# annihilatorrrr/spacedrive

Measured on AMD Instinct MI355X. Metric: cas_ids/sec + hashed GB/s (whole node), 10M files at 1/2/4/8 MI355X, higher is better.
Workload: dtype u32; 1 GPU; sampled-path cas_id (57,352-B BLAKE3 message/file) + Object grouping; 1310720 files/GPU/step (1310720 per step at n_gpus=1); dup_permille=300, parallelism=shard-by-file x1, grouping=fused

## Files before the change

spacedrive_amd/csrc/cas_hash.hip:

```cpp
#include <hip/hip_runtime.h>
#include <stdint.h>

#include "blake3_lane.hpp"
#include "blake3_tree.hpp"
#include "sd_dup_probe.h"
#include "sd_dup_runs.h"
#include "sd_group.h"
#include "sd_kernels.h"
#include "sd_mix.h"
#include "sd_ws.h"

namespace sdcas {


constexpr uint32_t SAMPLED_PAIRS = SAMPLED_CONTENT_LEN / 128;
constexpr uint32_t SAMPLED_CHUNKS = SAMPLED_CONTENT_LEN / 1024;
static_assert(SAMPLED_PAIRS == 8 * SAMPLED_CHUNKS, "the sampled content is whole chunks of 8 lines");

__device__ __forceinline__ void load_pair_here(const uint4* __restrict__ q, uint32_t P,
                                               uint4 (&buf)[8]) {
  __builtin_amdgcn_sched_barrier(0);
  line(q, P, buf);
  __builtin_amdgcn_sched_barrier(0);
}

constexpr int SAMPLED_DEPTH = 5;
constexpr int SAMPLED_BLOCK = 512;

template <int B = SAMPLED_BLOCK>
using LdsStack = CvStack<B, false>;

template <int BLK = SAMPLED_BLOCK>
__device__ __forceinline__ uint64_t cas_lane_sampled(const uint4* __restrict__ q, uint64_t size,
                                                     LdsStack<BLK>& stk) {
  uint4 A[8], B[8];
  uint32_t cv[8];
  auto push_chunk = [&](uint32_t total) { merge_push(stk, cv, total); };
// ... 136 lines not shown
  uint64_t key = 0;
  if (live) {
    LdsStack<B> stk{stack_lds, threadIdx.x};
    const uint4* q = reinterpret_cast<const uint4*>(content + f * stride);
    key = cas_lane_sampled<B>(q, sizes[f], stk);
  }
  if (blockIdx.x == 0 && threadIdx.x < 2) ro.objects[threadIdx.x] = 0;
  region_epilogue<B>(stack_lds, live, f, key, keys, ro);
}

extern "C" __global__ void __launch_bounds__(SAMPLED_BLOCK)
sd_cas_sampled_group_kernel(const uint8_t* __restrict__ content, uint64_t stride,
                            const uint64_t* __restrict__ sizes, uint64_t n,
                            uint64_t* __restrict__ keys, RegionOut ro) {
  sampled_group_kernel_body<SAMPLED_BLOCK>(content, stride, sizes, n, keys, ro);
}

extern "C" __global__ void __launch_bounds__(SAMPLED_BLOCK_NARROW)
sd_cas_sampled_group_kernel_256(const uint8_t* __restrict__ content, uint64_t stride,
                                const uint64_t* __restrict__ sizes, uint64_t n,
                                uint64_t* __restrict__ keys, RegionOut ro) {
  sampled_group_kernel_body<SAMPLED_BLOCK_NARROW>(content, stride, sizes, n, keys, ro);
}

struct DupLists {
  const uint32_t* cand;
  uint32_t* list_h;
  uint32_t* list_c;
  uint32_t* same;
  uint32_t* cnt;
  uint32_t* first;
  uint32_t* rank;
  uint32_t* counters;
  uint32_t tail_tiles;
  volatile uint32_t* note;
  uint32_t seq, files;
};
constexpr uint32_t DUP_N_HASH = 0, DUP_N_CAND = 1, DUP_VERIFIED = 2, DUP_REHASHED = 3, DUP_QUEUE = 4,
                   DUP_GROUPS = 5, DUP_TASKS = 6, DUP_REFS = 7;
static_assert(DUP_REFS < DUP_COUNTERS, "counters");

extern "C" __global__ void __launch_bounds__(256)
sd_dup_probe_kernel(const uint8_t* __restrict__ content, uint64_t stride,
                    const uint64_t* __restrict__ sizes, uint64_t n, uint64_t* __restrict__ probes,
                    uint32_t* __restrict__ counters, uint32_t* __restrict__ cnt) {
  const uint64_t f = (uint64_t)blockIdx.x * 256 + threadIdx.x;
  if (blockIdx.x == 0 && threadIdx.x < DUP_COUNTERS) counters[threadIdx.x] = 0;
  if (f < n) {
    probes[f] = dup_probe(sizes[f], content + f * stride);
    cnt[f] = 0;
  }
}

extern "C" __global__ void __launch_bounds__(256)
sd_dup_compact_kernel(uint64_t n, DupLists dl) {
  __shared__ uint32_t wcnt[3][4], base;
  const uint64_t f = (uint64_t)blockIdx.x * 256 + threadIdx.x;
  const uint32_t lane = threadIdx.x & 63u, w = threadIdx.x >> 6;
  const bool live = f < n;
  const uint32_t g = live ? dl.cand[f] : 0u;
  const bool h = live && g == (uint32_t)f;
  const bool c = live && !h;
  uint32_t r = 1;
  if (c) {
    r = atomicAdd(&dl.cnt[g], 1u);
    dl.rank[f] = r;
  }
  const uint64_t bh = __ballot(h), bc = __ballot(c), bg = __ballot(r == 0);
  const uint64_t below = (1ull << lane) - 1ull;
  if (lane == 0) {
    wcnt[0][w] = (uint32_t)__popcll(bh);
    wcnt[1][w] = (uint32_t)__popcll(bc);
    wcnt[2][w] = (uint32_t)__popcll(bg);
  }
  __syncthreads();
  if (threadIdx.x < 3) {
    constexpr uint32_t word[3] = {DUP_N_HASH, DUP_N_CAND, DUP_GROUPS};
    const uint32_t t = wcnt[threadIdx.x][0] + wcnt[threadIdx.x][1] + wcnt[threadIdx.x][2] +
                       wcnt[threadIdx.x][3];
    const uint32_t b = t ? atomicAdd(&dl.counters[word[threadIdx.x]], t) : 0u;
// ... 67 lines not shown
  for (uint32_t s = 0; s < DUP_SLICES && alive; ++s) {
    DupSlice ref, cur, nxt;
    uint32_t left = alive;
    uint32_t e = dup_first_bit(left);
    uint32_t fe = (uint32_t)__builtin_amdgcn_readlane((int)f, (int)e);
    uint32_t loaded = (uint32_t)__builtin_popcount(heads & ((2u << e) - 1u));
    dup_load_slice(ref, content, stride, (uint32_t)__builtin_amdgcn_readfirstlane((int)dl.cand[fe]), s, voff);
    dup_load_slice(cur, content, stride, fe, s, voff);
#pragma unroll 1
    for (;;) {
      left &= left - 1u;
      uint32_t e2 = 0;
      if (left) {
        e2 = dup_first_bit(left);
        fe = (uint32_t)__builtin_amdgcn_readlane((int)f, (int)e2);
        dup_load_slice(nxt, content, stride, fe, s, voff);
      }
      if (dup_slices_differ(ref, cur)) alive &= ~(1u << e);
      if (!left) break;
      e = e2;
      cur = nxt;
      const uint32_t run = (uint32_t)__builtin_popcount(heads & ((2u << e) - 1u));
      if (run != loaded) {
        loaded = run;
        dup_load_slice(ref, content, stride, (uint32_t)__builtin_amdgcn_readfirstlane((int)dl.cand[fe]), s, voff);
      }
    }
  }
  lane = dup_lane_of(voff);
  if (lane < m) dl.same[f] = (alive >> lane) & 1u;
  return runs;
}

template <int B>
__device__ __forceinline__ void dup_mixed_kernel_body(const uint8_t* __restrict__ content,
                                                      uint64_t stride,
                                                      const uint64_t* __restrict__ sizes,
                                                      uint64_t* __restrict__ keys, RegionOut ro,
                                                      DupLists dl) {
  __shared__ uint32_t stack_lds[SAMPLED_DEPTH][8][B];
  const uint32_t n_hash = dl.counters[DUP_N_HASH], n_cand = dl.counters[DUP_N_CAND];
  const uint32_t G = gridDim.x;
  const uint32_t TH = (n_hash + B - 1) / B;
  const DupTile tile = dup_tile_of(blockIdx.x, G, TH, dl.tail_tiles);
  if (blockIdx.x == 0 && threadIdx.x < 2) ro.objects[threadIdx.x] = 0;
  if (blockIdx.x == 0 && threadIdx.x == 0 && dl.note) {
    dl.note[1] = n_cand;
    dl.note[2] = dl.files;
    __threadfence_system();
    dl.note[0] = dl.seq;
  }
  if (!tile.compare) {
    const uint32_t i = tile.hash_tile * B + threadIdx.x;
    const bool live = i < n_hash;
    uint64_t f = 0, key = 0;
    if (live) {
      f = dl.list_h[i];
      LdsStack<B> stk{stack_lds, threadIdx.x};
      const uint4* q = reinterpret_cast<const uint4*>(content + f * stride);
      key = cas_lane_sampled<B>(q, sizes[f], stk);
    }
    region_epilogue<B>(stack_lds, live, f, key, keys, ro);
  } else {
    const uint32_t voff = dup_slice_quad_offset(0, 0, threadIdx.x & 63u);
    const uint32_t n_tasks = dup_task_count(n_cand);
    uint32_t done = 0, refs = 0;
    for (uint32_t k = 0; tile.tail || k < dup_tile_wave_tasks(); ++k) {
      uint32_t t = 0;
      if (voff == 0) t = atomicAdd(&dl.counters[DUP_QUEUE], 1u);
      t = __builtin_amdgcn_readfirstlane(t);
      if (t >= n_tasks) break;
      refs += dup_compare_task(content, stride, sizes, dl, t, n_cand, voff);
      ++done;
    }
    if (voff == 0 && done) {
      atomicAdd(&dl.counters[DUP_TASKS], done);
      atomicAdd(&dl.counters[DUP_REFS], refs);
    }
  }
}

extern "C" __global__ void __launch_bounds__(SAMPLED_BLOCK)
sd_cas_dup_mixed_kernel(const uint8_t* __restrict__ content, uint64_t stride,
                        const uint64_t* __restrict__ sizes, uint64_t* __restrict__ keys,
                        RegionOut ro, DupLists dl) {
  dup_mixed_kernel_body<SAMPLED_BLOCK>(content, stride, sizes, keys, ro, dl);
}

extern "C" __global__ void __launch_bounds__(SAMPLED_BLOCK_NARROW)
sd_cas_dup_mixed_kernel_256(const uint8_t* __restrict__ content, uint64_t stride,
                            const uint64_t* __restrict__ sizes, uint64_t* __restrict__ keys,
                            RegionOut ro, DupLists dl) {
  dup_mixed_kernel_body<SAMPLED_BLOCK_NARROW>(content, stride, sizes, keys, ro, dl);
}

extern "C" __global__ void __launch_bounds__(SAMPLED_BLOCK_NARROW)
sd_cas_dup_finish_kernel(const uint8_t* __restrict__ content, uint64_t stride,
                         const uint64_t* __restrict__ sizes, uint64_t* __restrict__ keys,
                         RegionOut ro, DupLists dl) {
  constexpr int B = SAMPLED_BLOCK_NARROW;
  __shared__ uint32_t stack_lds[SAMPLED_DEPTH][8][B];
  const uint32_t n_cand = dl.counters[DUP_N_CAND];
  if (blockIdx.x * B >= n_cand) return;
  const uint32_t i = blockIdx.x * B + threadIdx.x;
  const bool live = i < n_cand;
  uint64_t f = 0, key = 0;
  bool ok = false;
  if (live) {
    f = dl.list_c[i];
    ok = dl.same[f] != 0;
    if (ok) key = keys[dl.cand[f]];
  }
  const uint64_t verified = __ballot(ok), failed = __ballot(live && !ok);
  if ((threadIdx.x & 63u) == 0) {
    if (verified) atomicAdd(&dl.counters[DUP_VERIFIED], (uint32_t)__popcll(verified));
    if (failed) atomicAdd(&dl.counters[DUP_REHASHED], (uint32_t)__popcll(failed));
  }
  if (failed) {
    if (live && !ok) {
      LdsStack<B> stk{stack_lds, threadIdx.x};
      const uint4* q = reinterpret_cast<const uint4*>(content + f * stride);
      key = cas_lane_sampled<B>(q, sizes[f], stk);
    }
  }
  region_epilogue<B>(stack_lds, live, f, key, keys, ro);
}

constexpr int PACKED_DEPTH = 6;
constexpr int PACKED_LDS_DEPTH = PACKED_DEPTH - 1;
constexpr int PACKED_BLOCK = 256;

using PackedStack = CvStack<PACKED_BLOCK, true>;

constexpr int CP_MAX_CHUNKS = 104;

// ... 54 lines not shown
    stk.pop(cv);
    fold(stk, cv, whole ? (uint32_t)ROOT : 0u);
  }
  uint32_t count = whole ? 1u : (nchunks + cpl - 1u) / cpl;
  segment_merge<SEG, 1u>(cv, sl, count);
  if (f < n && sl == 0u) keys[f] = ok ? key_of(cv) : 0ull;
}

template <int SEG>
__global__ void __launch_bounds__(64)
sd_cas_chunkpar_kernel(const uint8_t* __restrict__ arena, const uint64_t* __restrict__ offs,
                       uint64_t stride, const uint32_t* __restrict__ lens, uint32_t fixed_len,
                       const uint64_t* __restrict__ sizes, uint64_t n,
                       const uint32_t* __restrict__ order, uint64_t* __restrict__ keys) {
  chunkpar_wave<SEG>(arena, offs, stride, lens, fixed_len, sizes, n, order, keys);
}

extern "C" __global__ void __launch_bounds__(PACKED_BLOCK)
sd_cas_packed_kernel(const uint8_t* __restrict__ arena, const uint64_t* __restrict__ offs,
                     const uint32_t* __restrict__ lens, const uint64_t* __restrict__ sizes,
                     const uint32_t* __restrict__ order, uint64_t n,
                     uint64_t* __restrict__ keys) {
  __shared__ uint32_t stack_lds[PACKED_LDS_DEPTH][8][PACKED_BLOCK];
  const uint64_t t = (uint64_t)blockIdx.x * PACKED_BLOCK + threadIdx.x;
  if (t >= n) return;
  const uint32_t f = order ? order[t] : (uint32_t)t;
  const uint4* q = reinterpret_cast<const uint4*>(arena + offs[f]);
  PackedStack stk{stack_lds, threadIdx.x};
  uint32_t cv[8];
  lane_message<PREFIXED>(q, lens[f], sizes[f], stk, cv);
  keys[f] = key_of(cv);
}

}

namespace sdcas {

#ifndef SD_K2_BLOCK_KEY
#define SD_K2_BLOCK_KEY 0
#endif
#ifndef SD_K2_KEY_SHIFT
#define SD_K2_KEY_SHIFT 0
#endif
constexpr uint32_t CHUNK_KEY_BITS = SD_K2_BLOCK_KEY ? 11 : 7;

extern "C" __global__ void __launch_bounds__(256)
sd_cas_length_keys(const uint32_t* __restrict__ lens, uint64_t n, uint64_t* __restrict__ out) {
  const uint64_t i = (uint64_t)blockIdx.x * blockDim.x + threadIdx.x;
  if (i < n) {
    const uint64_t units = SD_K2_BLOCK_KEY ? ((uint64_t)lens[i] + 8u + 63u) >> 6
                                           : ((uint64_t)lens[i] + 8u + 1023u) >> (10 + SD_K2_KEY_SHIFT);
    out[i] = ((1ull << CHUNK_KEY_BITS) - 1) - units;
  }
}

int length_key_bits(uint64_t) { return (int)CHUNK_KEY_BITS; }

hipError_t hash_sampled(const uint8_t* content, uint64_t stride, const uint64_t* sizes,
                        uint64_t n, uint64_t* keys, hipStream_t s, uint32_t cus) {
  if (n == 0) return hipSuccess;
  const uint64_t blocks = (n + SAMPLED_BLOCK - 1) / SAMPLED_BLOCK;
  const uint64_t quanta = cus ? (n + (uint64_t)cus * 256 - 1) / ((uint64_t)cus * 256) : 0;
  if (cus && (blocks < cus || (quanta & 1))) {
    const uint64_t nb = (n + SAMPLED_BLOCK_NARROW - 1) / SAMPLED_BLOCK_NARROW;
    sd_cas_sampled_kernel_256<<<(uint32_t)nb, SAMPLED_BLOCK_NARROW, 0, s>>>(content, stride, sizes,
                                                                           n, keys);
  } else {
    sd_cas_sampled_kernel<<<(uint32_t)blocks, SAMPLED_BLOCK, 0, s>>>(content, stride, sizes, n, keys);
  }
  return hipGetLastError();
}

hipError_t hash_sampled_regions(const uint8_t* content, uint64_t stride, const uint64_t* sizes,
                                uint64_t n, uint64_t* keys, uint32_t* rep, uint64_t* rkeys,
                                uint32_t* rfile, uint32_t* cursor, uint64_t cap, uint64_t* spill_keys,
                                uint32_t* spill_file, uint32_t* overflow, uint64_t* objects,
                                hipStream_t s, uint32_t cus) {
  if (n == 0) return hipSuccess;
  const RegionOut ro{rkeys, rfile, cursor, cap, spill_keys, spill_file, rep, overflow,
                     (unsigned long long*)objects};
  const uint64_t blocks = (n + SAMPLED_BLOCK - 1) / SAMPLED_BLOCK;
  const uint64_t quanta = cus ? (n + (uint64_t)cus * 256 - 1) / ((uint64_t)cus * 256) : 0;
  if (cus && (blocks < cus || (quanta & 1))) {
    const uint64_t nb = (n + SAMPLED_BLOCK_NARROW - 1) / SAMPLED_BLOCK_NARROW;
    sd_cas_sampled_group_kernel_256<<<(uint32_t)nb, SAMPLED_BLOCK_NARROW, 0, s>>>(content, stride,
                                                                                 sizes, n, keys, ro);
  } else {
    sd_cas_sampled_group_kernel<<<(uint32_t)blocks, SAMPLED_BLOCK, 0, s>>>(content, stride, sizes, n,
                                                                          keys, ro);
  }
  return hipGetLastError();
}

DupVerifyWs dup_verify_layout(void* ws, uint64_t n) {
  WsCarve w(ws);  DupVerifyWs L;
  L.probes = w.take<uint64_t>(n);  L.cand = w.take<uint32_t>(n);
  L.list_h = w.take<uint32_t>(n);  L.list_c = w.take<uint32_t>(n);  L.same = w.take<uint32_t>(n);
  L.cnt = w.take<uint32_t>(n);  L.first = w.take<uint32_t>(n);  L.rank = w.take<uint32_t>(n);
  L.partial = w.take<uint32_t>(n / 4096 + 1);
  L.counters = w.take<uint32_t>(DUP_COUNTERS);  L.objects = w.take<uint64_t>(1);
  L.bytes = w.bytes();  return L;
}
size_t dup_verify_workspace_bytes(uint64_t n) { return dup_verify_layout(nullptr, n).bytes; }

#ifndef SD_DUP_TAIL_NUM
#define SD_DUP_TAIL_NUM 5u
#define SD_DUP_TAIL_DEN 7u
#endif

hipError_t dup_candidates(const uint8_t* content, uint64_t stride, const uint64_t* sizes, uint64_t n,
                          const DupVerifyWs& L, void* group_ws, uint32_t* totals, hipStream_t s) {
  if (n == 0) return hipSuccess;
  sd_dup_probe_kernel<<<(uint32_t)((n + 255) / 256), 256, 0, s>>>(content, stride, sizes, n, L.probes,
                                                                  L.counters, L.cnt);
  hipError_t e = hipGetLastError();
  if (e != hipSuccess) return e;
  return hash_group_min(L.probes, nullptr, n, L.cand, L.objects, group_ws, totals, s);
}

hipError_t hash_sampled_regions_verify(const uint8_t* content, uint64_t stride, const uint64_t* sizes,
                                       uint64_t n, uint64_t* keys, uint32_t* rep, uint64_t* rkeys,
                                       uint32_t* rfile, uint32_t* cursor, uint64_t cap,
                                       uint64_t* spill_keys, uint32_t* spill_file, uint32_t* overflow,
                                       uint64_t* objects, const DupVerifyWs& L, uint32_t* note,
                                       uint32_t seq, hipStream_t s, uint32_t cus) {
  if (n == 0) return hipSuccess;
  const RegionOut ro{rkeys, rfile, cursor, cap, spill_keys, spill_file, rep, overflow,
                     (unsigned long long*)objects};
  const uint64_t blocks = (n + SAMPLED_BLOCK - 1) / SAMPLED_BLOCK;
  const uint64_t quanta = cus ? (n + (uint64_t)cus * 256 - 1) / ((uint64_t)cus * 256) : 0;
  const bool narrow = cus && (blocks < cus || (quanta & 1));
  const uint32_t slots = (cus ? cus : 256u) * (narrow ? 4u : 2u);
  const uint32_t tail_tiles = slots * SD_DUP_TAIL_NUM / SD_DUP_TAIL_DEN;
  const DupLists dl{L.cand, L.list_h, L.list_c, L.same, L.cnt, L.first, L.rank, L.counters,
                    tail_tiles, note, seq, (uint32_t)n};
  const uint32_t nb256 = (uint32_t)((n + 255) / 256);
  sd_dup_compact_kernel<<<nb256, 256, 0, s>>>(n, dl);
  hipError_t e = exclusive_scan_u32(L.cnt, L.first, n, L.partial, s);
  if (e != hipSuccess) return e;
  sd_dup_order_kernel<<<nb256, 256, 0, s>>>(n, dl);
  if (narrow) {
    const uint64_t nb = (n + SAMPLED_BLOCK_NARROW - 1) / SAMPLED_BLOCK_NARROW;
    sd_cas_dup_mixed_kernel_256<<<(uint32_t)nb + 1, SAMPLED_BLOCK_NARROW, 0, s>>>(content, stride, sizes,
                                                                                 keys, ro, dl);
  } else {
    sd_cas_dup_mixed_kernel<<<(uint32_t)blocks + 1, SAMPLED_BLOCK, 0, s>>>(content, stride, sizes, keys,
                                                                          ro, dl);
  }
  const uint64_t fb = (n + SAMPLED_BLOCK_NARROW - 1) / SAMPLED_BLOCK_NARROW;
  sd_cas_dup_finish_kernel<<<(uint32_t)fb, SAMPLED_BLOCK_NARROW, 0, s>>>(content, stride, sizes, keys,
                                                                        ro, dl);
  return hipGetLastError();
}

#ifndef SD_PULL_UNROLL
#define SD_PULL_UNROLL 4
#endif
#ifndef SD_PULL_WIDE_BYTES
#define SD_PULL_WIDE_BYTES (512u << 10)
#endif
template <int U>
__global__ void __launch_bounds__(256)
sd_pull_host(const uint4* __restrict__ src, uint4* __restrict__ dst, uint64_t quads) {
  const uint64_t step = (uint64_t)gridDim.x * 256;
  for (uint64_t i = (uint64_t)blockIdx.x * 256 + threadIdx.x; i < quads; i += step * U) {
    uint4 v[U];
#pragma unroll
    for (int u = 0; u < U; ++u)
      if (i + u * step < quads) v[u] = src[i + u * step];
#pragma unroll
    for (int u = 0; u < U; ++u)
      if (i + u * step < quads) dst[i + u * step] = v[u];
  }
}

hipError_t pull_host(void* dst, const void* src, uint64_t bytes, hipStream_t s) {
// ... 46 lines not shown
```

spacedrive_amd/csrc/ctx_internal.h:

```cpp
#pragma once
#include <hip/hip_runtime.h>
#include <dirent.h>
#include <pthread.h>
#include <sched.h>
#include <stdarg.h>
#include <stdio.h>
#include <stdlib.h>
#include <string.h>
#include <sys/syscall.h>
#include <unistd.h>

#include <algorithm>
#include <atomic>
#include <chrono>
#include <condition_variable>
#include <functional>
#include <mutex>
#include <string>
#include <thread>
#include <vector>

#include "../../include/sd_hip_cas.h"
#include "sd_debug.h"
#include "sd_ws.h"
// ... 69 lines not shown
  void loop() {
    if (private_fds_ && access("/proc/thread-self/fd", R_OK) == 0 && unshare(CLONE_FILES) == 0) {
      keep_only_device_fds();
      nprivate_.fetch_add(1);
    }
    uint64_t seen = 0;
    std::unique_lock<std::mutex> lk(mu_);
    for (;;) {
      cv_.wait(lk, [&] { return stop_ || (gen_ != seen && want_ > 0); });
      if (stop_) return;
      seen = gen_;
      --want_;
      const std::function<void()>* f = fn_;
      lk.unlock();
      (*f)();
      lk.lock();
      if (--pending_ == 0) done_.notify_one();
    }
  }
  std::mutex mu_;
  std::condition_variable cv_, done_;
  std::vector<std::thread> th_;
  const std::function<void()>* fn_ = nullptr;
  unsigned want_ = 0, pending_ = 0;
  uint64_t gen_ = 0;
  bool stop_ = false;
  cpu_set_t cpus_{};
  int ncpus_ = 0;
  bool private_fds_ = false;
  std::atomic<int> nprivate_{0};
};

constexpr uint32_t DUPV_SKIP_CALLS = 16, DUPV_MIN_CANDIDATE_SHARE = 32;

struct sd_cas_ctx {
  int device = 0;
  hipStream_t stream = nullptr;
  hipStream_t copy = nullptr;
  hipStream_t copy2 = nullptr;
  hipEvent_t copy2_done = nullptr;
  hipEvent_t h2d_done = nullptr;
  hipEvent_t packed_h2d = nullptr;
  hipEvent_t packed_done = nullptr;
  DevBuf ws;
  DevBuf staging;
  DevBuf small;
  DevBuf cvbuf;
  DevBuf io;
  DevBuf inplace;
  DevBuf dupv;
  DevBuf exact;
  int exact_method = 0;
  uint64_t exact_mismatched = 0, exact_fallbacks = 0;
  bool dup_verify = true;
  uint64_t dupv_n = 0;
  hipStream_t dupv_stream = nullptr;
  uint32_t* dupv_note = nullptr;
  uint32_t dupv_seq = 0;
  uint32_t dupv_seen = 0;
  uint32_t dupv_skip = 0;
  void* pinned = nullptr;
  size_t pinned_bytes = 0;
  uint64_t* d_scalar = nullptr;
  uint32_t* gtotals = nullptr;
  uint32_t* gcursor = nullptr;
  DevBuf regions[2];
  uint64_t region_n[2] = {0, 0};
  const uint64_t* region_keys[2] = {nullptr, nullptr};
  hipEvent_t region_done[2] = {nullptr, nullptr};
  hipEvent_t region_hashed[2] = {nullptr, nullptr};
  bool region_pending[2] = {false, false};
  bool region_grouped[2] = {true, true};
  int region_cur = -1;
  int region_obj_set = -1;
  hipEvent_t ws_ev = nullptr;
  hipStream_t ws_stream = nullptr;
  bool ws_pending = false;
  size_t quantum = 65536;
  int group_method = 0;
  uint64_t group_target = 0;
  bool use_hash_group(uint64_t n) const {
    return group_method == SD_CAS_GROUP_HASH ||
           (group_method == SD_CAS_GROUP_AUTO && n <= SD_CAS_HASH_GROUP_MAX_KEYS);
  }
  size_t latency_sampled = 0, latency_packed = 0;
  size_t seg16_sampled = 0, seg16_packed = 0;
  int chunkpar_seg(size_t n, bool sampled) const {
// ... 195 lines not shown
```

spacedrive_amd/csrc/sd_dup_runs.h:

```cpp
#pragma once
#include <stdint.h>

#if defined(__HIPCC__)
#define SD_RUNS_HD __host__ __device__
#else
#define SD_RUNS_HD
#endif

namespace sdcas {

#ifndef SD_DUP_RUN_K
#define SD_DUP_RUN_K 16
#endif
constexpr uint32_t DUP_RUN_K = SD_DUP_RUN_K;
static_assert(DUP_RUN_K >= 1 && DUP_RUN_K <= 32, "a task's entries are the bits of one u32");

constexpr uint32_t DUP_ROW_BYTES = 57344;
constexpr uint32_t DUP_WAVE = 64;
constexpr uint32_t DUP_SLICE_QUADS = 8;
constexpr uint32_t DUP_SLICE_BYTES = DUP_WAVE * DUP_SLICE_QUADS * 16;
constexpr uint32_t DUP_SLICES = DUP_ROW_BYTES / DUP_SLICE_BYTES;
static_assert(DUP_SLICES * DUP_SLICE_BYTES == DUP_ROW_BYTES, "a row is whole slices");

SD_RUNS_HD inline uint32_t dup_task_count(uint32_t n_cand) {
  return n_cand / DUP_RUN_K + (n_cand % DUP_RUN_K ? 1u : 0u);
}
SD_RUNS_HD inline uint32_t dup_task_first(uint32_t t) { return t * DUP_RUN_K; }
SD_RUNS_HD inline uint32_t dup_task_entries(uint32_t t, uint32_t n_cand) {
  const uint32_t left = n_cand - dup_task_first(t);
  return left < DUP_RUN_K ? left : DUP_RUN_K;
}

struct DupTile {
  bool compare, tail;
  uint32_t hash_tile;
};
SD_RUNS_HD inline DupTile dup_tile_of(uint32_t b, uint32_t G, uint32_t TH, uint32_t tail_tiles) {
  const uint32_t TC = G - TH;
  const uint32_t TT = TC < tail_tiles ? TC : tail_tiles;
  const uint32_t GI = G - TT, TI = TC - TT;
  if (b >= GI) return {true, true, 0u};
  const uint32_t c0 = (uint32_t)((uint64_t)b * TI / GI);
  const uint32_t c1 = (uint32_t)(((uint64_t)b + 1) * TI / GI);
  return {c0 != c1, false, b - c0};
}
SD_RUNS_HD inline uint32_t dup_tile_wave_tasks(void) { return (DUP_WAVE + DUP_RUN_K - 1) / DUP_RUN_K; }

SD_RUNS_HD inline uint32_t dup_slice_quad_offset(uint32_t s, uint32_t u, uint32_t lane) {
  return s * DUP_SLICE_BYTES + (u * DUP_WAVE + lane) * 16u;
}

}
```

spacedrive_amd/csrc/sd_hip_cas.cpp:

```cpp
#include <ctype.h>
#include <errno.h>
#include <fcntl.h>
#include <hip/hip_runtime.h>
#include <stdarg.h>
#include <stdio.h>
#include <stdlib.h>
#include <string.h>
#include <sys/stat.h>
#include <unistd.h>

#include <algorithm>
#include <atomic>
#include <memory>
#include <string>
#include <thread>
#include <vector>

#include "sd_checksum.h"
#include "sd_exact_dups.h"
#include "sd_group.h"
#include "sd_kernels.h"
#include "sd_links.h"
#include "sd_mix.h"
#include "sd_object_stats.h"
#include "sd_synth.h"

using namespace sdcas;

#include "sd_debug.h"
#if SD_DBG
namespace sdcas {
uint32_t sd_dbg_violations_group_hash();
uint32_t sd_dbg_violations_group();
uint32_t sd_dbg_violations_checksum();
uint32_t sd_dbg_violations_links();
uint32_t sd_dbg_violations_inplace();
uint32_t sd_dbg_violations_object_stats();
uint32_t sd_dbg_violations_exact_dups();
}
#include "ctx_internal.h"
extern "C" uint64_t sd_cas_debug_violations(void) {
  return (uint64_t)sd_dbg_violations_group_hash() + sd_dbg_violations_group() +
         sd_dbg_violations_checksum() + sd_dbg_violations_links() + sd_dbg_violations_inplace() +
         sd_dbg_violations_object_stats() + sd_dbg_violations_exact_dups() + sd_dbg_tail_check_all();
}

namespace {
struct DbgTail { void* p; size_t bytes; std::string name; int device; };
std::mutex g_tail_mu;
std::vector<DbgTail> g_tails;
uint64_t g_tail_violations = 0;

inline uint8_t tail_byte(size_t i) { return (uint8_t)((i * 167u + 13u) ^ (i >> 8) ^ 0xA5u); }
const uint8_t* tail_pattern() {
  static uint8_t pat[SD_DBG_TAIL_BYTES];
  static bool made = false;
  if (!made) {
    for (size_t i = 0; i < sizeof pat; i++) pat[i] = tail_byte(i);
    made = true;
  }
  return pat;
}
void tail_check_one(const DbgTail& t, const char* when) {
  uint8_t got[SD_DBG_TAIL_BYTES];
  uint8_t* tail = (uint8_t*)t.p + up256(t.bytes);
  if (hipMemcpy(got, tail, sizeof got, hipMemcpyDeviceToHost) != hipSuccess) {
    (void)hipGetLastError();
    ++g_tail_violations;
    printf("SD_CAS tail of %s (%zu bytes) could not be read (%s)\n", t.name.c_str(), t.bytes, when);
    fflush(stdout);
    return;
  }
  const uint8_t* pat = tail_pattern();
  if (memcmp(got, pat, sizeof got) == 0) return;
  size_t first = 0, changed = 0;
// ... 139 lines not shown
      hipStreamCreateWithFlags(&c->copy2, hipStreamNonBlocking) != hipSuccess ||
      hipEventCreateWithFlags(&c->copy2_done, hipEventDisableTiming) != hipSuccess ||
      hipEventCreateWithFlags(&c->h2d_done, hipEventDisableTiming) != hipSuccess ||
      hipEventCreateWithFlags(&c->packed_h2d, hipEventDisableTiming) != hipSuccess ||
      hipEventCreateWithFlags(&c->packed_done, hipEventDisableTiming) != hipSuccess ||
      hipEventCreateWithFlags(&c->ws_ev, hipEventDisableTiming) != hipSuccess ||
      sd_dev_malloc((void**)&c->d_scalar, 64, "d_scalar") != hipSuccess ||
      hipHostMalloc((void**)&c->dupv_note, 64, hipHostMallocDefault) != hipSuccess ||
      sd_dev_malloc((void**)&c->gtotals, GROUP_TOTALS_WORDS * 4, "gtotals") != hipSuccess ||
      hipMemset(c->gtotals, 0, GROUP_TOTALS_WORDS * 4) != hipSuccess ||
      sd_dev_malloc((void**)&c->gcursor, 2 * REGION_SET_WORDS * 4, "gcursor") != hipSuccess ||
      hipMemset(c->gcursor, 0, 2 * REGION_SET_WORDS * 4) != hipSuccess ||
      hipEventCreateWithFlags(&c->region_done[0], hipEventDisableTiming) != hipSuccess ||
      hipEventCreateWithFlags(&c->region_done[1], hipEventDisableTiming) != hipSuccess ||
      hipEventCreateWithFlags(&c->region_hashed[0], hipEventDisableTiming) != hipSuccess ||
      hipEventCreateWithFlags(&c->region_hashed[1], hipEventDisableTiming) != hipSuccess ||
      hipEventCreateWithFlags(&c->gather_done[0], hipEventDisableTiming) != hipSuccess ||
      hipEventCreateWithFlags(&c->gather_done[1], hipEventDisableTiming) != hipSuccess) {
    sd_cas_ctx_destroy(c);
    g_ctx_create_err = "stream/event/scratch creation failed on device " + std::to_string(device);
    return SD_CAS_EHIP;
  }
  memset(c->dupv_note, 0, 64);
  c->quantum = (size_t)prop.multiProcessorCount * 4 * 64;
  {
    const char* t = getenv("SD_CAS_TRACE");
    c->trace = t && *t && strcmp(t, "0") != 0;
    const char* f = getenv("SD_CAS_TEST_TABLE_FILL");
    c->test_table_fill = f && *f ? (uint32_t)strtoul(f, nullptr, 10) : 0u;
    if (c->test_table_fill)
      fprintf(stderr, "sd_hip_cas: SD_CAS_TEST_TABLE_FILL=%u (test knob): the fused grouping's "
              "region tables overflow at %u distinct keys (exact, much slower)\n",
              c->test_table_fill, c->test_table_fill);
  }
  bind_pool_to_gpu_node(c);
  const char* pf = getenv("SD_CAS_POOL_PRIVATE_FDS");
  const bool private_fds = !(pf && pf[0] == '0');
  c->pool.set_private_fds(private_fds);
  if (c->trace)
    fprintf(stderr, "sd_cas_trace ctx device=%d numa_node=%d pool_cpus=%d private_fds=%d\n", device,
            c->numa_node, c->pool.bound_cpus(), (int)private_fds);
  sd_cas_set_latency_threshold(c, SD_CAS_THRESHOLD_DEFAULT, SD_CAS_THRESHOLD_DEFAULT);
  sd_cas_set_chunkpar_split(c, SD_CAS_THRESHOLD_DEFAULT, SD_CAS_THRESHOLD_DEFAULT);
  *out = c;
  return SD_CAS_OK;
}

void sd_cas_set_latency_threshold(sd_cas_ctx* c, size_t sampled_files, size_t packed_files) {
  if (!c) return;
  const size_t q = sd_cas_batch_quantum(c);
  c->latency_sampled = sampled_files == SD_CAS_THRESHOLD_DEFAULT ? q * 3 / 4 : sampled_files;
  c->latency_packed = packed_files == SD_CAS_THRESHOLD_DEFAULT ? q * 2 : packed_files;
}

void sd_cas_set_chunkpar_split(sd_cas_ctx* c, size_t sampled_files, size_t packed_files) {
  if (!c) return;
  const size_t q = sd_cas_batch_quantum(c);
  c->seg16_sampled = sampled_files == SD_CAS_THRESHOLD_DEFAULT ? q * 3 / 64 : sampled_files;
  c->seg16_packed = packed_files == SD_CAS_THRESHOLD_DEFAULT ? q * 3 / 32 : packed_files;
}

void sd_cas_ctx_destroy(sd_cas_ctx* c) {
  if (!c) return;
  (void)hipSetDevice(c->device);
  (void)hipDeviceSynchronize();
  if (c->ws.p) (void)sd_dev_free(c->ws.p);
// ... 237 lines not shown
    HIP_TRY(c, sd_ws_acquire(c, s));
    HIP_TRY(c, hipMemcpyAsync(c->d_scalar, region_group_layout(c->regions[k].p, c->region_n[k]).objects, 8,
                              hipMemcpyDeviceToDevice, s));
    HIP_TRY(c, sd_ws_release(c, s));
    c->region_obj_set = -1;
  }
  c->region_n[k] = n;
  int rc = ensure(c, c->regions[k], region_group_workspace_bytes(n));
  if (rc) return rc;
  const RegionGroupWs L = region_group_layout(c->regions[k].p, c->region_n[k]);
  uint32_t* cur = c->gcursor + REGION_SET_WORDS * k;
  hipError_t e;
  bool verify = c->dup_verify;
  if (verify && c->dupv_skip) {
    c->dupv_skip--;
    verify = false;
  } else if (verify) {
    const volatile uint32_t* note = c->dupv_note;
    const uint32_t seq = note[0], cand = note[1], files = note[2];
    if (seq != c->dupv_seen && note[0] == seq) {
      c->dupv_seen = seq;
      if ((uint64_t)cand * DUPV_MIN_CANDIDATE_SHARE < files) {
        c->dupv_skip = DUPV_SKIP_CALLS - 1;
        verify = false;
      }
    }
  }
  if (verify) {
    if ((rc = ensure(c, c->dupv, dup_verify_workspace_bytes(n)))) return rc;
    if ((rc = ensure(c, c->ws, hash_group_workspace_bytes(n)))) return rc;
    if (c->dupv_n && c->dupv_stream != s && c->region_cur >= 0)
      HIP_TRY(c, hipStreamWaitEvent(s, c->region_hashed[c->region_cur], 0));
    const DupVerifyWs D = dup_verify_layout(c->dupv.p, n);
    HIP_TRY(c, sd_ws_acquire(c, s));
    e = dup_candidates((const uint8_t*)d_content, stride, d_sizes, n, D, c->ws.p, c->gtotals, s);
    HIP_TRY(c, sd_ws_release(c, s));
    if (e == hipSuccess)
      e = hash_sampled_regions_verify((const uint8_t*)d_content, stride, d_sizes, n, d_keys, d_rep,
                                      L.rkeys, L.rfile, cur, region_capacity(n), L.spill_keys,
                                      L.spill_file, d_overflow, L.objects, D, c->dupv_note,
                                      ++c->dupv_seq, s, (uint32_t)(c->quantum / 256));
    c->dupv_n = e == hipSuccess ? n : 0;
    c->dupv_stream = s;
  } else {
    e = hash_sampled_regions((const uint8_t*)d_content, stride, d_sizes, n, d_keys, d_rep,
                             L.rkeys, L.rfile, cur, region_capacity(n), L.spill_keys,
                             L.spill_file, d_overflow, L.objects, s, (uint32_t)(c->quantum / 256));
    c->dupv_n = 0;
  }
  if (e != hipSuccess) {
    (void)hipMemsetAsync(cur, 0, REGION_SET_WORDS * 4, s);
    return fail(c, SD_CAS_EHIP, "hash_regions: %s", hipGetErrorString(e));
  }
  HIP_TRY(c, hipEventRecord(c->region_hashed[k], s));
  c->region_keys[k] = d_keys;
  c->region_cur = k;
  c->region_grouped[k] = false;
  return SD_CAS_OK;
}

static int dup_verify_words(sd_cas_ctx* c, uint32_t (&h)[DUP_COUNTERS]) {
  if (c->dupv_n && c->region_cur >= 0) {
    HIP_TRY(c, hipSetDevice(c->device));
    HIP_TRY(c, hipStreamWaitEvent(c->stream, c->region_hashed[c->region_cur], 0));
    HIP_TRY(c, hipMemcpyAsync(h, dup_verify_layout(c->dupv.p, c->dupv_n).counters, sizeof h,
                              hipMemcpyDeviceToHost, c->stream));
    HIP_TRY(c, hipStreamSynchronize(c->stream));
  }
  return SD_CAS_OK;
}

int sd_cas_dup_verify_counters(sd_cas_ctx* c, uint64_t* out_candidates, uint64_t* out_verified,
                               uint64_t* out_rehashed) {
  if (!c || !out_candidates || !out_verified || !out_rehashed) return SD_CAS_EINVAL;
// ... 830 lines not shown
```

spacedrive_amd/csrc/sd_kernels.h:

```cpp
#pragma once
#include <stdint.h>

namespace sdcas {

constexpr uint64_t SAMPLE_COUNT = 4;
constexpr uint64_t SAMPLE_SIZE = 1024 * 10;
constexpr uint64_t HEADER_OR_FOOTER_SIZE = 1024 * 8;
constexpr uint64_t MINIMUM_FILE_SIZE = 1024 * 100;
constexpr uint32_t SAMPLED_CONTENT_LEN =
    (uint32_t)(2 * HEADER_OR_FOOTER_SIZE + SAMPLE_COUNT * SAMPLE_SIZE);
static_assert(2 * HEADER_OR_FOOTER_SIZE + SAMPLE_COUNT * SAMPLE_SIZE < MINIMUM_FILE_SIZE, "cas.rs:18");
static_assert(SAMPLE_SIZE > HEADER_OR_FOOTER_SIZE, "cas.rs:21");

constexpr uint32_t MAX_PACKED_CONTENT_LEN = 104u * 1024u - 8u;

}

#include <hip/hip_runtime.h>
namespace sdcas {
hipError_t hash_sampled(const uint8_t* content, uint64_t stride, const uint64_t* sizes,
                        uint64_t n, uint64_t* keys, hipStream_t s, uint32_t cus);
hipError_t hash_sampled_regions(const uint8_t* content, uint64_t stride, const uint64_t* sizes,
                                uint64_t n, uint64_t* keys, uint32_t* rep, uint64_t* rkeys,
                                uint32_t* rfile, uint32_t* cursor, uint64_t cap, uint64_t* spill_keys,
                                uint32_t* spill_file, uint32_t* overflow, uint64_t* objects,
                                hipStream_t s, uint32_t cus);
constexpr uint32_t DUP_COUNTERS = 8;
struct DupVerifyWs {
  uint64_t* probes; uint32_t *cand, *list_h, *list_c, *same, *cnt, *first, *rank, *partial, *counters;
  uint64_t* objects; size_t bytes;
};
DupVerifyWs dup_verify_layout(void* ws, uint64_t n);
size_t dup_verify_workspace_bytes(uint64_t n);
hipError_t dup_candidates(const uint8_t* content, uint64_t stride, const uint64_t* sizes, uint64_t n,
                          const DupVerifyWs& L, void* group_ws, uint32_t* totals, hipStream_t s);
hipError_t hash_sampled_regions_verify(const uint8_t* content, uint64_t stride, const uint64_t* sizes,
                                       uint64_t n, uint64_t* keys, uint32_t* rep, uint64_t* rkeys,
                                       uint32_t* rfile, uint32_t* cursor, uint64_t cap,
                                       uint64_t* spill_keys, uint32_t* spill_file, uint32_t* overflow,
                                       uint64_t* objects, const DupVerifyWs& L, uint32_t* note,
                                       uint32_t seq, hipStream_t s, uint32_t cus);
hipError_t pull_host(void* dst, const void* src, uint64_t bytes, hipStream_t s);
hipError_t hash_packed(const uint8_t* arena, const uint64_t* offs, const uint32_t* lens,
                       const uint64_t* sizes, const uint32_t* order, uint64_t n, uint64_t* keys,
                       hipStream_t s);
hipError_t length_keys(const uint32_t* lens, uint64_t n, uint64_t* out, hipStream_t s);
hipError_t hash_chunkpar(const uint8_t* arena, const uint64_t* offs, uint64_t stride,
                         const uint32_t* lens, uint32_t fixed_len, const uint64_t* sizes,
                         uint64_t n, uint64_t* keys, int seg, hipStream_t s,
                         const uint32_t* order = nullptr);
int length_key_bits(uint64_t n);
struct InplaceWs { uint32_t *counters, *lens32, *sampled_idx; size_t bytes; };
InplaceWs inplace_layout(void* ws, uint64_t n);
size_t inplace_workspace_bytes(uint64_t n);
hipError_t inplace_classify(uint64_t arena_bytes, const uint64_t* offs, const uint64_t* lens,
                            uint64_t n, void* ws, hipStream_t s);
hipError_t hash_inplace_sampled(const uint8_t* arena, const uint64_t* offs, const uint64_t* lens,
                                const uint32_t* idx, uint64_t n_idx, uint64_t* keys,
                                hipStream_t s);
}
```

Baseline: 62.79 million cas_ids/s.

## Assign hash/compare roles dynamically per workgroup with per-CU compare limits

Replaces the static blockIdx-based split between hash tiles and duplicate-compare tasks in the mixed kernel with runtime role claiming. Each workgroup reads the hash and compare queues, and takes a compare role only if compares are not ahead of hashing and its CU (found through the hardware ID registers) has no other compare workgroup. Otherwise it claims the next hash tile. The goal is to balance the two kinds of work and keep memory-bound compares from piling onto one CU. The cost is extra atomics and per-CU counters, and the narrow 256-thread kernel is forced whenever roles are enabled. An auto heuristic turns roles on for large grids.

```diff
diff --git a/spacedrive_amd/csrc/cas_hash.hip b/spacedrive_amd/csrc/cas_hash.hip
--- a/spacedrive_amd/csrc/cas_hash.hip
+++ b/spacedrive_amd/csrc/cas_hash.hip
@@ -3,6 +3,7 @@
 
 #include "blake3_lane.hpp"
 #include "blake3_tree.hpp"
+#include "sd_debug.h"
 #include "sd_dup_probe.h"
 #include "sd_dup_runs.h"
 #include "sd_group.h"
@@ -205,20 +206,26 @@
   uint32_t* first;
   uint32_t* rank;
   uint32_t* counters;
+  uint32_t* cu;
   uint32_t tail_tiles;
+  uint32_t slots;
   volatile uint32_t* note;
   uint32_t seq, files;
 };
 constexpr uint32_t DUP_N_HASH = 0, DUP_N_CAND = 1, DUP_VERIFIED = 2, DUP_REHASHED = 3, DUP_QUEUE = 4,
-                   DUP_GROUPS = 5, DUP_TASKS = 6, DUP_REFS = 7;
-static_assert(DUP_REFS < DUP_COUNTERS, "counters");
+                   DUP_GROUPS = 5, DUP_TASKS = 6, DUP_REFS = 7, DUP_HASH_QUEUE = 8, DUP_COMPARE_WGS = 9,
+                   DUP_TILES_RUN = 10, DUP_TILES_WANT = 11;
+static_assert(DUP_TILES_RUN < DUP_TILES_WANT && DUP_TILES_WANT < DUP_COUNTERS, "counters");
 
 extern "C" __global__ void __launch_bounds__(256)
 sd_dup_probe_kernel(const uint8_t* __restrict__ content, uint64_t stride,
                     const uint64_t* __restrict__ sizes, uint64_t n, uint64_t* __restrict__ probes,
-                    uint32_t* __restrict__ counters, uint32_t* __restrict__ cnt) {
+                    uint32_t* __restrict__ counters, uint32_t* __restrict__ cu,
+                    uint32_t* __restrict__ cnt) {
   const uint64_t f = (uint64_t)blockIdx.x * 256 + threadIdx.x;
   if (blockIdx.x == 0 && threadIdx.x < DUP_COUNTERS) counters[threadIdx.x] = 0;
+  if (blockIdx.x == 0)
+    for (uint32_t i = threadIdx.x; i < DUP_CU_SLOTS; i += 256) cu[i] = 0;
   if (f < n) {
     probes[f] = dup_probe(sizes[f], content + f * stride);
     cnt[f] = 0;
@@ -352,6 +359,12 @@
   return runs;
 }
 
+__device__ __forceinline__ uint32_t dup_this_cu_slot() {
+  constexpr int HW_REG_HW_ID = 4, HW_REG_XCC_ID = 20, WHOLE = 31 << 11;
+  return dup_cu_slot(__builtin_amdgcn_s_getreg(HW_REG_XCC_ID | WHOLE),
+                     __builtin_amdgcn_s_getreg(HW_REG_HW_ID | WHOLE));
+}
+
 template <int B>
 __device__ __forceinline__ void dup_mixed_kernel_body(const uint8_t* __restrict__ content,
                                                       uint64_t stride,
@@ -362,7 +375,45 @@
   const uint32_t n_hash = dl.counters[DUP_N_HASH], n_cand = dl.counters[DUP_N_CAND];
   const uint32_t G = gridDim.x;
   const uint32_t TH = (n_hash + B - 1) / B;
-  const DupTile tile = dup_tile_of(blockIdx.x, G, TH, dl.tail_tiles);
+  DupTile tile;
+  uint32_t quota = dup_tile_wave_tasks();
+  bool leaves_cu = false;
+  const bool roles = B == (int)DUP_ROLE_BLOCK && dl.tail_tiles == 0;
+  if (roles) {
+    const uint32_t n_tasks = dup_task_count(n_cand);
+    if (threadIdx.x == 0) {
+      uint32_t role = DUP_ROLE_COMPARE;
+      bool compare = dup_wants_compare(
+          __hip_atomic_load(&dl.counters[DUP_QUEUE], __ATOMIC_RELAXED, __HIP_MEMORY_SCOPE_AGENT), n_tasks,
+          __hip_atomic_load(&dl.counters[DUP_HASH_QUEUE], __ATOMIC_RELAXED, __HIP_MEMORY_SCOPE_AGENT), TH);
+      if (compare) {
+        const uint32_t slot = dup_this_cu_slot();
+        compare = dup_cu_has_room(atomicAdd(&dl.cu[slot], 1u)) &&
+                  atomicAdd(&dl.counters[DUP_COMPARE_WGS], 1u) < dup_compare_budget(G, TH);
+        if (!compare) atomicSub(&dl.cu[slot], 1u);
+        stack_lds[0][0][1] = slot;
+      }
+      if (!compare) {
+        role = atomicAdd(&dl.counters[DUP_HASH_QUEUE], 1u);
+        if (role >= TH) role = DUP_ROLE_DRAIN;
+      }
+      stack_lds[0][0][0] = role;
+    }
+    __syncthreads();
+    const uint32_t role = (uint32_t)__builtin_amdgcn_readfirstlane((int)stack_lds[0][0][0]);
+    __syncthreads();
+    tile = DupTile{role >= DUP_ROLE_COMPARE, role == DUP_ROLE_DRAIN || !dup_compare_has_quota(G, dl.slots), role};
+    quota = dup_role_wave_tasks();
+    leaves_cu = role == DUP_ROLE_COMPARE;
+  } else {
+    tile = dup_tile_of(blockIdx.x, G, TH, dl.tail_tiles);
+  }
+#if SD_DBG
+  if (threadIdx.x == 0) {
+    if (blockIdx.x == 0) dl.counters[DUP_TILES_WANT] = TH;
+    if (!tile.compare) atomicAdd(&dl.counters[DUP_TILES_RUN], 1u);
+  }
+#endif
   if (blockIdx.x == 0 && threadIdx.x < 2) ro.objects[threadIdx.x] = 0;
   if (blockIdx.x == 0 && threadIdx.x == 0 && dl.note) {
     dl.note[1] = n_cand;
@@ -385,7 +436,7 @@
     const uint32_t voff = dup_slice_quad_offset(0, 0, threadIdx.x & 63u);
     const uint32_t n_tasks = dup_task_count(n_cand);
     uint32_t done = 0, refs = 0;
-    for (uint32_t k = 0; tile.tail || k < dup_tile_wave_tasks(); ++k) {
+    for (uint32_t k = 0; tile.tail || k < quota; ++k) {
       uint32_t t = 0;
       if (voff == 0) t = atomicAdd(&dl.counters[DUP_QUEUE], 1u);
       t = __builtin_amdgcn_readfirstlane(t);
@@ -396,6 +447,10 @@
     if (voff == 0 && done) {
       atomicAdd(&dl.counters[DUP_TASKS], done);
       atomicAdd(&dl.counters[DUP_REFS], refs);
+    }
+    if (leaves_cu) {
+      __syncthreads();
+      if (threadIdx.x == 0) atomicSub(&dl.cu[stack_lds[0][0][1]], 1u);
     }
   }
 }
@@ -421,6 +476,16 @@
   constexpr int B = SAMPLED_BLOCK_NARROW;
   __shared__ uint32_t stack_lds[SAMPLED_DEPTH][8][B];
   const uint32_t n_cand = dl.counters[DUP_N_CAND];
+#if SD_DBG
+  if (blockIdx.x == 0) {
+    SD_DBG_CHECK(threadIdx.x != 0 || dl.counters[DUP_TILES_RUN] == dl.counters[DUP_TILES_WANT],
+                 "dup roles: %u hash tiles run of %u", dl.counters[DUP_TILES_RUN], dl.counters[DUP_TILES_WANT]);
+    SD_DBG_CHECK(threadIdx.x != 0 || dl.counters[DUP_TASKS] == dup_task_count(n_cand),
+                 "dup roles: %u tasks run of %u", dl.counters[DUP_TASKS], dup_task_count(n_cand));
+    for (uint32_t i = threadIdx.x; i < DUP_CU_SLOTS; i += B)
+      SD_DBG_CHECK(dl.cu[i] == 0, "dup roles: CU slot %u left at %u", i, dl.cu[i]);
+  }
+#endif
   if (blockIdx.x * B >= n_cand) return;
   const uint32_t i = blockIdx.x * B + threadIdx.x;
   const bool live = i < n_cand;
@@ -541,6 +606,8 @@
   keys[f] = key_of(cv);
 }
 
+SD_DBG_ACCESSOR(sd_dbg_violations_cas_hash)
+
 }
 
 namespace sdcas {
@@ -607,7 +674,8 @@
   L.list_h = w.take<uint32_t>(n);  L.list_c = w.take<uint32_t>(n);  L.same = w.take<uint32_t>(n);
   L.cnt = w.take<uint32_t>(n);  L.first = w.take<uint32_t>(n);  L.rank = w.take<uint32_t>(n);
   L.partial = w.take<uint32_t>(n / 4096 + 1);
-  L.counters = w.take<uint32_t>(DUP_COUNTERS);  L.objects = w.take<uint64_t>(1);
+  L.counters = w.take<uint32_t>(DUP_COUNTERS);  L.cu = w.take<uint32_t>(DUP_CU_SLOTS);
+  L.objects = w.take<uint64_t>(1);
   L.bytes = w.bytes();  return L;
 }
 size_t dup_verify_workspace_bytes(uint64_t n) { return dup_verify_layout(nullptr, n).bytes; }
@@ -621,7 +689,7 @@
                           const DupVerifyWs& L, void* group_ws, uint32_t* totals, hipStream_t s) {
   if (n == 0) return hipSuccess;
   sd_dup_probe_kernel<<<(uint32_t)((n + 255) / 256), 256, 0, s>>>(content, stride, sizes, n, L.probes,
-                                                                  L.counters, L.cnt);
+                                                                  L.counters, L.cu, L.cnt);
   hipError_t e = hipGetLastError();
   if (e != hipSuccess) return e;
   return hash_group_min(L.probes, nullptr, n, L.cand, L.objects, group_ws, totals, s);
@@ -632,25 +700,25 @@
                                        uint32_t* rfile, uint32_t* cursor, uint64_t cap,
                                        uint64_t* spill_keys, uint32_t* spill_file, uint32_t* overflow,
                                        uint64_t* objects, const DupVerifyWs& L, uint32_t* note,
-                                       uint32_t seq, hipStream_t s, uint32_t cus) {
+                                       uint32_t seq, hipStream_t s, uint32_t cus, bool cu_roles) {
   if (n == 0) return hipSuccess;
   const RegionOut ro{rkeys, rfile, cursor, cap, spill_keys, spill_file, rep, overflow,
                      (unsigned long long*)objects};
   const uint64_t blocks = (n + SAMPLED_BLOCK - 1) / SAMPLED_BLOCK;
   const uint64_t quanta = cus ? (n + (uint64_t)cus * 256 - 1) / ((uint64_t)cus * 256) : 0;
-  const bool narrow = cus && (blocks < cus || (quanta & 1));
+  const bool narrow = cu_roles || (cus && (blocks < cus || (quanta & 1)));
   const uint32_t slots = (cus ? cus : 256u) * (narrow ? 4u : 2u);
-  const uint32_t tail_tiles = slots * SD_DUP_TAIL_NUM / SD_DUP_TAIL_DEN;
-  const DupLists dl{L.cand, L.list_h, L.list_c, L.same, L.cnt, L.first, L.rank, L.counters,
-                    tail_tiles, note, seq, (uint32_t)n};
+  const uint32_t tail_tiles = cu_roles ? 0u : slots * SD_DUP_TAIL_NUM / SD_DUP_TAIL_DEN;
+  const DupLists dl{L.cand, L.list_h, L.list_c, L.same, L.cnt, L.first, L.rank, L.counters, L.cu,
+                    tail_tiles, slots, note, seq, (uint32_t)n};
   const uint32_t nb256 = (uint32_t)((n + 255) / 256);
   sd_dup_compact_kernel<<<nb256, 256, 0, s>>>(n, dl);
   hipError_t e = exclusive_scan_u32(L.cnt, L.first, n, L.partial, s);
   if (e != hipSuccess) return e;
   sd_dup_order_kernel<<<nb256, 256, 0, s>>>(n, dl);
   if (narrow) {
-    const uint64_t nb = (n + SAMPLED_BLOCK_NARROW - 1) / SAMPLED_BLOCK_NARROW;
-    sd_cas_dup_mixed_kernel_256<<<(uint32_t)nb + 1, SAMPLED_BLOCK_NARROW, 0, s>>>(content, stride, sizes,
+    static_assert(SAMPLED_BLOCK_NARROW == (int)DUP_ROLE_BLOCK, "dup_role_grid is this grid");
+    sd_cas_dup_mixed_kernel_256<<<dup_role_grid(n), SAMPLED_BLOCK_NARROW, 0, s>>>(content, stride, sizes,
                                                                                  keys, ro, dl);
   } else {
     sd_cas_dup_mixed_kernel<<<(uint32_t)blocks + 1, SAMPLED_BLOCK, 0, s>>>(content, stride, sizes, keys,
diff --git a/spacedrive_amd/csrc/ctx_internal.h b/spacedrive_amd/csrc/ctx_internal.h
--- a/spacedrive_amd/csrc/ctx_internal.h
+++ b/spacedrive_amd/csrc/ctx_internal.h
@@ -125,6 +125,7 @@
 };
 
 constexpr uint32_t DUPV_SKIP_CALLS = 16, DUPV_MIN_CANDIDATE_SHARE = 32;
+enum DupPlacement { DUP_PLACE_STATIC = 0, DUP_PLACE_CU = 1, DUP_PLACE_AUTO = 2 };
 
 struct sd_cas_ctx {
   int device = 0;
@@ -146,6 +147,7 @@
   int exact_method = 0;
   uint64_t exact_mismatched = 0, exact_fallbacks = 0;
   bool dup_verify = true;
+  DupPlacement dup_placement = DUP_PLACE_AUTO;
   uint64_t dupv_n = 0;
   hipStream_t dupv_stream = nullptr;
   uint32_t* dupv_note = nullptr;
diff --git a/spacedrive_amd/csrc/sd_dup_runs.h b/spacedrive_amd/csrc/sd_dup_runs.h
--- a/spacedrive_amd/csrc/sd_dup_runs.h
+++ b/spacedrive_amd/csrc/sd_dup_runs.h
@@ -46,6 +46,47 @@
 }
 SD_RUNS_HD inline uint32_t dup_tile_wave_tasks(void) { return (DUP_WAVE + DUP_RUN_K - 1) / DUP_RUN_K; }
 
+constexpr uint32_t DUP_ROLE_BLOCK = 256;
+#ifndef SD_DUP_CU_LIMIT
+#define SD_DUP_CU_LIMIT 1
+#endif
+#ifndef SD_DUP_QUOTA_MUL
+#define SD_DUP_QUOTA_MUL 1
+#endif
+constexpr uint32_t DUP_CU_LIMIT = SD_DUP_CU_LIMIT;
+constexpr uint32_t DUP_QUOTA_MUL = SD_DUP_QUOTA_MUL;
+static_assert(DUP_QUOTA_MUL >= 1, "a compare workgroup covers at least one tile's worth of list C");
+
+constexpr uint32_t DUP_CU_SLOTS = 16u * 256u;
+SD_RUNS_HD inline uint32_t dup_cu_slot(uint32_t xcc_id_reg, uint32_t hw_id_reg) {
+  return ((xcc_id_reg & 15u) << 8) | ((hw_id_reg >> 8) & 255u);
+}
+SD_RUNS_HD inline uint32_t dup_role_grid(uint64_t n) {
+  return (uint32_t)((n + DUP_ROLE_BLOCK - 1) / DUP_ROLE_BLOCK) + 1u;
+}
+SD_RUNS_HD inline uint32_t dup_role_hash_tiles(uint32_t n_hash) {
+  return n_hash / DUP_ROLE_BLOCK + (n_hash % DUP_ROLE_BLOCK ? 1u : 0u);
+}
+SD_RUNS_HD inline uint32_t dup_role_wave_tasks(void) { return dup_tile_wave_tasks() * DUP_QUOTA_MUL; }
+SD_RUNS_HD inline bool dup_compare_has_quota(uint32_t G, uint32_t slots) { return G > slots; }
+constexpr uint32_t DUP_ROLES_MIN_ROUNDS = 3;
+SD_RUNS_HD inline bool dup_roles_pay(uint32_t G, uint32_t slots) {
+  return (uint64_t)G >= (uint64_t)DUP_ROLES_MIN_ROUNDS * slots;
+}
+SD_RUNS_HD inline uint32_t dup_compare_budget(uint32_t G, uint32_t TH) { return G - TH; }
+SD_RUNS_HD inline bool dup_compares_not_ahead(uint32_t tasks_taken, uint32_t tasks_total,
+                                              uint32_t tiles_taken, uint32_t tiles_total) {
+  return (uint64_t)tasks_taken * tiles_total <= (uint64_t)tiles_taken * tasks_total;
+}
+SD_RUNS_HD inline bool dup_wants_compare(uint32_t task_queue, uint32_t tasks_total, uint32_t hash_queue,
+                                         uint32_t tiles_total) {
+  if (task_queue >= tasks_total) return false;
+  const uint32_t tiles_taken = hash_queue < tiles_total ? hash_queue : tiles_total;
+  return dup_compares_not_ahead(task_queue, tasks_total, tiles_taken, tiles_total);
+}
+SD_RUNS_HD inline bool dup_cu_has_room(uint32_t cu_compare) { return DUP_CU_LIMIT == 0 || cu_compare < DUP_CU_LIMIT; }
+constexpr uint32_t DUP_ROLE_COMPARE = 0x80000000u, DUP_ROLE_DRAIN = 0xC0000000u;
+
 SD_RUNS_HD inline uint32_t dup_slice_quad_offset(uint32_t s, uint32_t u, uint32_t lane) {
   return s * DUP_SLICE_BYTES + (u * DUP_WAVE + lane) * 16u;
 }
diff --git a/spacedrive_amd/csrc/sd_hip_cas.cpp b/spacedrive_amd/csrc/sd_hip_cas.cpp
--- a/spacedrive_amd/csrc/sd_hip_cas.cpp
+++ b/spacedrive_amd/csrc/sd_hip_cas.cpp
@@ -19,6 +19,7 @@
 #include "sd_checksum.h"
 #include "sd_exact_dups.h"
 #include "sd_group.h"
+#include "sd_dup_runs.h"
 #include "sd_kernels.h"
 #include "sd_links.h"
 #include "sd_mix.h"
@@ -31,6 +32,7 @@
 #if SD_DBG
 namespace sdcas {
 uint32_t sd_dbg_violations_group_hash();
+uint32_t sd_dbg_violations_cas_hash();
 uint32_t sd_dbg_violations_group();
 uint32_t sd_dbg_violations_checksum();
 uint32_t sd_dbg_violations_links();
@@ -40,7 +42,7 @@
 }
 #include "ctx_internal.h"
 extern "C" uint64_t sd_cas_debug_violations(void) {
-  return (uint64_t)sd_dbg_violations_group_hash() + sd_dbg_violations_group() +
+  return (uint64_t)sd_dbg_violations_group_hash() + sd_dbg_violations_cas_hash() + sd_dbg_violations_group() +
          sd_dbg_violations_checksum() + sd_dbg_violations_links() + sd_dbg_violations_inplace() +
          sd_dbg_violations_object_stats() + sd_dbg_violations_exact_dups() + sd_dbg_tail_check_all();
 }
@@ -246,6 +248,15 @@
       fprintf(stderr, "sd_hip_cas: SD_CAS_TEST_TABLE_FILL=%u (test knob): the fused grouping's "
               "region tables overflow at %u distinct keys (exact, much slower)\n",
               c->test_table_fill, c->test_table_fill);
+    const char* p = getenv("SD_CAS_DUP_PLACEMENT");
+    if (p && *p) {
+      if (strcmp(p, "cu") != 0 && strcmp(p, "static") != 0 && strcmp(p, "auto") != 0) {
+        sd_cas_ctx_destroy(c);
+        g_ctx_create_err = std::string("SD_CAS_DUP_PLACEMENT=") + p + ": static, cu or auto";
+        return SD_CAS_EINVAL;
+      }
+      c->dup_placement = !strcmp(p, "cu") ? DUP_PLACE_CU : !strcmp(p, "static") ? DUP_PLACE_STATIC : DUP_PLACE_AUTO;
+    }
   }
   bind_pool_to_gpu_node(c);
   const char* pf = getenv("SD_CAS_POOL_PRIVATE_FDS");
@@ -549,6 +560,9 @@
     if (c->dupv_n && c->dupv_stream != s && c->region_cur >= 0)
       HIP_TRY(c, hipStreamWaitEvent(s, c->region_hashed[c->region_cur], 0));
     const DupVerifyWs D = dup_verify_layout(c->dupv.p, n);
+    const uint32_t cus = (uint32_t)(c->quantum / 256);
+    const bool cu_roles = c->dup_placement == DUP_PLACE_CU ||
+                          (c->dup_placement == DUP_PLACE_AUTO && dup_roles_pay(dup_role_grid(n), 4 * cus));
     HIP_TRY(c, sd_ws_acquire(c, s));
     e = dup_candidates((const uint8_t*)d_content, stride, d_sizes, n, D, c->ws.p, c->gtotals, s);
     HIP_TRY(c, sd_ws_release(c, s));
@@ -556,7 +570,7 @@
       e = hash_sampled_regions_verify((const uint8_t*)d_content, stride, d_sizes, n, d_keys, d_rep,
                                       L.rkeys, L.rfile, cur, region_capacity(n), L.spill_keys,
                                       L.spill_file, d_overflow, L.objects, D, c->dupv_note,
-                                      ++c->dupv_seq, s, (uint32_t)(c->quantum / 256));
+                                      ++c->dupv_seq, s, cus, cu_roles);
     c->dupv_n = e == hipSuccess ? n : 0;
     c->dupv_stream = s;
   } else {
diff --git a/spacedrive_amd/csrc/sd_kernels.h b/spacedrive_amd/csrc/sd_kernels.h
--- a/spacedrive_amd/csrc/sd_kernels.h
+++ b/spacedrive_amd/csrc/sd_kernels.h
@@ -25,9 +25,9 @@
                                 uint32_t* rfile, uint32_t* cursor, uint64_t cap, uint64_t* spill_keys,
                                 uint32_t* spill_file, uint32_t* overflow, uint64_t* objects,
                                 hipStream_t s, uint32_t cus);
-constexpr uint32_t DUP_COUNTERS = 8;
+constexpr uint32_t DUP_COUNTERS = 16;
 struct DupVerifyWs {
-  uint64_t* probes; uint32_t *cand, *list_h, *list_c, *same, *cnt, *first, *rank, *partial, *counters;
+  uint64_t* probes; uint32_t *cand, *list_h, *list_c, *same, *cnt, *first, *rank, *partial, *counters, *cu;
   uint64_t* objects; size_t bytes;
 };
 DupVerifyWs dup_verify_layout(void* ws, uint64_t n);
@@ -39,7 +39,7 @@
                                        uint32_t* rfile, uint32_t* cursor, uint64_t cap,
                                        uint64_t* spill_keys, uint32_t* spill_file, uint32_t* overflow,
                                        uint64_t* objects, const DupVerifyWs& L, uint32_t* note,
-                                       uint32_t seq, hipStream_t s, uint32_t cus);
+                                       uint32_t seq, hipStream_t s, uint32_t cus, bool cu_roles);
 hipError_t pull_host(void* dst, const void* src, uint64_t bytes, hipStream_t s);
 hipError_t hash_packed(const uint8_t* arena, const uint64_t* offs, const uint32_t* lens,
                        const uint64_t* sizes, const uint32_t* order, uint64_t n, uint64_t* keys,
```

New measurement: 67.86 million cas_ids/s (median of 6 runs). 1.08x the previous value.
